# lixiaobai09/xgnn

Measured on AMD Instinct MI355X. Metric: sampled edges/s + feature-extract GB/s per epoch-step, higher is better.
Workload: dtype u32 ids / f32 rows (bit copy)

## Files before the change

### include/ggms.h

```cpp
#ifndef GGMS_H
#define GGMS_H

#include <stddef.h>
#include <stdint.h>

#ifdef __cplusplus
extern "C" {
#endif

typedef uint32_t ggms_id_t;
typedef void *ggms_stream_t;
typedef void *ggms_event_t;
#define GGMS_EMPTY_KEY 0xffffffffu

enum ggms_status {
  GGMS_OK = 0,
  GGMS_ERR_INVALID = -1,
  GGMS_ERR_HIP = -2,
  GGMS_ERR_NO_DEVICE = -3
};

enum ggms_dtype {
  GGMS_F32 = 0,
  GGMS_F64 = 1,
// ... 8 lines not shown
  GGMS_Q8ROW = 18
};

int ggms_abi_version(void);
const char *ggms_last_error(void);

#define GGMS_STATUS_SCAN_SPIN 1u
#define GGMS_STATUS_TABLE_FULL 2u
#define GGMS_STATUS_PREFETCH_FULL 4u
int ggms_device_status(uint32_t *status_host, int clear);
#define GGMS_PROBE_ATOMIC 0
#define GGMS_PROBE_LOAD 1
#define GGMS_PROBE_LOAD_ATOMIC 2
int ggms_fabric_probe(int kind, void *table, size_t table_words, size_t num_requests, uint32_t salt, void *sink,
                      ggms_stream_t stream);
void ggms_debug_poison_next_scan(void);
void ggms_debug_set_scan_patience(uint32_t polls);
void ggms_debug_delay_next_scan(uint32_t sleeps);
uint32_t ggms_debug_set_scan_epoch(uint32_t counter);
#define GGMS_DEBUG_KHOP0_DRAW_CAP 0
#define GGMS_DEBUG_OWNER_SCAN_CHUNKS 1
#define GGMS_DEBUG_OWNER_SCAN_TILES 2
#define GGMS_DEBUG_GRID_CAP 3
#define GGMS_DEBUG_NUM_KNOBS 4
void ggms_debug_set_knob(int knob, long long value);
size_t ggms_dtype_bytes(int dtype);
size_t ggms_row_bytes(int dtype, size_t dim);

#define GGMS_MAX_PARTS 8
typedef struct {
  const ggms_id_t *indptr;
  const ggms_id_t *indices;
  const ggms_id_t *const *part_indptr;
  const ggms_id_t *const *part_indices;
  uint32_t num_part;
  uint32_t num_cache_node;
  uint32_t num_node;
  uint32_t heads_id;
} ggms_graph_t;

#define GGMS_LIST_HEAD_BYTES 64
#define GGMS_LIST_HEAD_INLINE 15
#define GGMS_LIST_HEADS_MAX 255
size_t ggms_list_heads_bytes(size_t num_node);
int ggms_list_heads_build(const ggms_graph_t *graph, void *heads, size_t bytes, ggms_stream_t stream);
int ggms_list_heads_attach(ggms_graph_t *graph, const void *heads);
int ggms_list_heads_detach(ggms_graph_t *graph);
const void *ggms_list_heads_of(const ggms_graph_t *graph);
// ... 487 lines not shown
```

### xgnn_amd/_lib.py

```python
import ctypes as C
import os

_HERE = os.path.dirname(os.path.abspath(__file__))
LIB_PATH = os.path.join(_HERE, "lib", "libggms_hip.so")
_LIB = None


class GgmsError(RuntimeError):
    pass


class Graph(C.Structure):
    _fields_ = [("indptr", C.c_void_p), ("indices", C.c_void_p),
                ("part_indptr", C.c_void_p), ("part_indices", C.c_void_p),
                ("num_part", C.c_uint32), ("num_cache_node", C.c_uint32),
                ("num_node", C.c_uint32), ("heads_id", C.c_uint32)]


class SampleExtra(C.Structure):
    _fields_ = [("prob_table", C.c_void_p), ("alias_table", C.c_void_p), ("random_walk_length", C.c_size_t),
                ("random_walk_restart_prob", C.c_double), ("num_random_walk", C.c_size_t), ("data", C.c_void_p),
                ("rng_wait", C.c_void_p), ("rng_done", C.c_void_p), ("heavy_wait", C.c_void_p),
                ("seeds_distinct", C.c_uint32), ("labor_salt", C.c_uint32)]

# ... 57 lines not shown


class Topology(C.Structure):
    _fields_ = [("num_device", C.c_int32), ("_pad", C.c_int32), ("can_access", (C.c_int32 * 16) * 16),
                ("copy_GBps", (C.c_double * 16) * 16)]


class HashTable(C.Structure):
    _fields_ = [("o2n", C.c_void_p), ("n2o", C.c_void_p), ("num_items_dev", C.c_void_p),
                ("o2n_size", C.c_uint64), ("n2o_size", C.c_uint64),
                ("version", C.c_uint32), ("direct", C.c_uint32)]


_vp, _sz, _u64, _u32, _i = C.c_void_p, C.c_size_t, C.c_uint64, C.c_uint32, C.c_int
SYMBOLS = {
    "ggms_abi_version": (_i, []),
    "ggms_last_error": (C.c_char_p, []),
    "ggms_device_status": (_i, [C.POINTER(_u32), _i]),
    "ggms_debug_poison_next_scan": (None, []),
    "ggms_debug_set_scan_patience": (None, [C.c_uint32]),
    "ggms_debug_delay_next_scan": (None, [C.c_uint32]),
    "ggms_debug_set_scan_epoch": (C.c_uint32, [C.c_uint32]),
    "ggms_debug_set_knob": (None, [_i, C.c_longlong]),
    "ggms_fabric_probe": (_i, [_i, _vp, _sz, _sz, _u32, _vp, _vp]),
    "ggms_dtype_bytes": (_sz, [_i]),
    "ggms_row_bytes": (_sz, [_i, _sz]),
    "ggms_list_heads_bytes": (_sz, [_sz]),
    "ggms_list_heads_build": (_i, [C.POINTER(Graph), _vp, _sz, _vp]),
    "ggms_list_heads_attach": (_i, [C.POINTER(Graph), _vp]),
    "ggms_list_heads_detach": (_i, [C.POINTER(Graph)]),
    "ggms_list_heads_of": (_vp, [C.POINTER(Graph)]),
    "ggms_random_states_init": (_i, [_vp, _sz, _u64, _vp]),
    "ggms_random_states_count": (_sz, [_i, C.POINTER(_sz), _sz, _sz, _sz]),
    "ggms_sample_workspace_bytes": (_sz, [_i, _sz, _sz]),
    "ggms_sample_khop3": (_i, [C.POINTER(Graph), _vp, _sz, _sz, _vp, _vp, _vp, _vp, _sz, _vp, _sz, _vp]),
    "ggms_sample_khop0": (_i, [C.POINTER(Graph), _vp, _sz, _sz, _vp, _vp, _vp, _vp, _sz, _vp]),
    "ggms_sample_khop_labor": (_i, [C.POINTER(Graph), _vp, _sz, _sz, C.c_uint32, _vp, _vp, _vp, _vp, _sz, _vp]),
    "ggms_sample_khop_temporal": (_i, [C.POINTER(Graph), _vp, _vp, _vp, _sz, _sz, _i, C.c_uint32, _vp, _vp, _vp, _vp, _vp,
                                       _sz, _vp]),
    "ggms_sample_khop1": (_i, [C.POINTER(Graph), _vp, _sz, _sz, _vp, _vp, _vp, _vp, _sz, _vp, _sz, _vp]),
    "ggms_sample_khop2": (_i, [C.POINTER(Graph), _vp, _sz, _sz, _vp, _vp, _vp, _vp, _sz, _vp, _sz, _vp]),
    "ggms_sample_weighted_workspace_bytes": (_sz, [_sz, _sz]),
    "ggms_sample_weighted_khop": (_i, [C.POINTER(Graph), _vp, _vp, _vp, _sz, _sz, _vp, _vp, _vp, _vp, _sz, _vp, _sz,
                                       _vp]),
    "ggms_sample_weighted_khop_prefix": (_i, [C.POINTER(Graph), _vp, _vp, _sz, _sz, _vp, _vp, _vp, _vp, _sz, _vp, _sz,
                                              _vp]),
# ... 133 lines not shown
```

### xgnn_amd/csrc/common.hip

```cpp
#include <atomic>
#include <cstdarg>
#include <cstdio>
#include <mutex>
#include <random>

#include "row_formats.h"
#include "tile_scan.h"

namespace ggms {

static thread_local char g_err[512] = "";

void set_error(const char *fmt, ...) {
  va_list ap;
  va_start(ap, fmt);
  vsnprintf(g_err, sizeof(g_err), fmt, ap);
  va_end(ap);
}

uint32_t *device_status_word() {
  static std::mutex mu;
  static uint32_t *words[64] = {nullptr};
  int dev = 0;
  if (hipGetDevice(&dev) != hipSuccess || dev < 0 || dev >= 64) return nullptr;
  std::lock_guard<std::mutex> lock(mu);
  if (!words[dev]) {
    uint32_t *p = nullptr;
    if (hipMalloc((void **)&p, 64) != hipSuccess) return nullptr;
    if (hipMemset(p, 0, 64) != hipSuccess) {
      (void)hipFree(p);
      return nullptr;
    }
    words[dev] = p;
  }
  return words[dev];
}

size_t device_lds_bytes() {
  int dev = 0, v = 0;
  if (hipGetDevice(&dev) != hipSuccess) return 0;
  if (hipDeviceGetAttribute(&v, hipDeviceAttributeMaxSharedMemoryPerBlock, dev) != hipSuccess || v <= 0) return 0;
  return (size_t)v;
}

int raise_dynamic_lds(const void *func, size_t bytes, const char *who) {
  const size_t have = device_lds_bytes();
  if (have != 0 && bytes > have) {
    set_error("%s needs %zu bytes of LDS per workgroup, this device offers %zu: the library is built for gfx950 (160 KB)",
              who, bytes, have);
    return GGMS_ERR_INVALID;
  }
  GGMS_HIP(hipFuncSetAttribute(func, hipFuncAttributeMaxDynamicSharedMemorySize, (int)bytes));
  return GGMS_OK;
}

bool host_readable_table(const void *table, const char *what) {
  static thread_local const void *last_ok[2] = {nullptr, nullptr};
  if (table == last_ok[0] || table == last_ok[1]) return true;
  struct Remember {
    const void *t;
    bool ok = true;
    ~Remember() { if (ok) { last_ok[1] = last_ok[0]; last_ok[0] = t; } }
  } remember{table};
  hipPointerAttribute_t a;
  if (hipPointerGetAttributes(&a, table) != hipSuccess) {
    (void)hipGetLastError();
    return true;
  }
  if (a.type == hipMemoryTypeDevice) {
    set_error("%s is a DEVICE pointer: since ABI 3 the shard pointer tables are HOST arrays (include/ggms.h)", what);
    remember.ok = false;
    return false;
  }
  return true;
}

std::atomic<long long> &debug_knob_word(int knob) {
  static std::atomic<long long> v[GGMS_DEBUG_NUM_KNOBS] = {{-1}, {-1}, {-1}, {-1}};
  return v[knob];
}
long long debug_knob(int knob) { return debug_knob_word(knob).load(std::memory_order_relaxed); }

unsigned long long next_dedup_tag() {
  static std::atomic<unsigned long long> g{[] {
    std::random_device rd;
    return (((unsigned long long)rd() << 32) | rd()) | 1ull;
  }()};
  return g.fetch_add(1) + 1;
}

__global__ __launch_bounds__(kBlock) void k_init_states(uint32_t *states, uint64_t num, uint64_t seed) {
  for (uint64_t t = (uint64_t)blockIdx.x * kBlock + threadIdx.x; t < num; t += (uint64_t)gridDim.x * kBlock) {
    Xorwow st;
    st.init(seed + t);
    st.store(states + 6 * t);
  }
}

}

using namespace ggms;

extern "C" {

int ggms_abi_version(void) { return 3; }

void ggms_debug_set_knob(int knob, long long value) {
  if (knob >= 0 && knob < GGMS_DEBUG_NUM_KNOBS) debug_knob_word(knob).store(value < 0 ? -1 : value);
}

int ggms_device_status(uint32_t *status_host, int clear) {
  GGMS_CHECK_ARG(status_host);
  uint32_t *w = device_status_word();
  if (!w) {
    set_error("ggms_device_status: no device status word (no device?)");
    return GGMS_ERR_NO_DEVICE;
  }
  GGMS_HIP(hipDeviceSynchronize());
  GGMS_HIP(hipMemcpy(status_host, w, sizeof(uint32_t), hipMemcpyDeviceToHost));
  if (clear && *status_host) {
    GGMS_HIP(hipMemset(w, 0, sizeof(uint32_t)));
    GGMS_HIP(hipDeviceSynchronize());
  }
  return GGMS_OK;
}

const char *ggms_last_error(void) { return g_err; }

size_t ggms_dtype_bytes(int dtype) {
  switch (dtype) {
    case GGMS_F32: return 4;
    case GGMS_F64: return 8;
    case GGMS_F16: return 2;
    case GGMS_U8: return 1;
    case GGMS_I32: return 4;
    case GGMS_I8: return 1;
    case GGMS_I64: return 8;
    case GGMS_BF16: return 2;
    case GGMS_F8E4M3: return 1;
    case GGMS_F8E5M2: return 1;
    default: return 0;
  }
}

// ... 50 lines not shown
```

### xgnn_amd/csrc/ggms_device.h

```cpp
#pragma once
#include <cstdlib>

#include <hip/hip_runtime.h>
#include <stdint.h>

#include "../../include/ggms.h"

namespace ggms {

constexpr uint32_t kEmptyKey = GGMS_EMPTY_KEY;
constexpr int kWave = 64;
constexpr int kBlock = 256;
constexpr int kMaxGridBlocks = 2048;

void set_error(const char *fmt, ...);
#define GGMS_CHECK_ARG(cond)                                              \
  do {                                                                    \
    if (!(cond)) {                                                        \
      ::ggms::set_error("%s:%d: invalid argument: %s", __FILE__, __LINE__, #cond); \
      return GGMS_ERR_INVALID;                                            \
    }                                                                     \
  } while (0)
#define GGMS_HIP(call)                                                    \
  do {                                                                    \
// ... 194 lines not shown
  unsigned long long *w;
  uint32_t version;
  uint32_t *cand;
  unsigned long long *lost;
  unsigned long long tag;
  uint32_t base;
  uint32_t batch;
  IdxMap map;
  __device__ __forceinline__ unsigned long long issue(uint32_t key, uint32_t e) const {
    return atomicMin(w + key, make_w1(version, 1u, base + e));
  }
  __device__ __forceinline__ void enter(uint32_t key, uint32_t e) const { finish(issue(key, e), e); }
  __device__ __forceinline__ void finish(unsigned long long old, uint32_t e) const {
    const unsigned long long mine = make_w1(version, 1u, base + e);
    if (old > mine) {
      cand[e] = 1u;
      if ((old >> 32) == (mine >> 32)) lost[(uint32_t)old - base] = tag;
    } else {
      const uint32_t idx = (uint32_t)old;
      cand[e] = (batch && idx < base) ? 2u + map.local_of(idx) : 0u;
    }
  }
};
unsigned long long next_dedup_tag();
size_t device_lds_bytes();
int raise_dynamic_lds(const void *func, size_t bytes, const char *who);

__device__ __forceinline__ uint32_t lane_id() { return threadIdx.x & 63u; }

__device__ __forceinline__ uint64_t shfl_u64(uint64_t v, int src) {
  const uint32_t lo = __shfl((uint32_t)v, src, 64);
  const uint32_t hi = __shfl((uint32_t)(v >> 32), src, 64);
  return ((uint64_t)hi << 32) | lo;
}

__device__ __forceinline__ uint32_t wave_inclusive_scan(uint32_t x) {
#pragma unroll
  for (int off = 1; off < 64; off <<= 1) {
    const uint32_t y = __shfl_up(x, off, 64);
    if ((int)lane_id() >= off) x += y;
  }
  return x;
}

__device__ __forceinline__ uint32_t wave_reduce_sum(uint32_t x) {
#pragma unroll
// ... 23 lines not shown
```

### xgnn_amd/csrc/ggms_internal.h

```cpp
#pragma once
#include "tile_scan.h"

namespace ggms {

struct SrcMode {
  const uint32_t *seed_local;
  int local;
  __device__ __forceinline__ uint32_t value(uint32_t rid, uint64_t index) const {
    if (!local) return rid;
    return seed_local ? seed_local[index] : (uint32_t)index;
  }
};

struct BatchPrologue {
  uint32_t *zero_words;
  uint32_t num_zero;
  uint32_t *zero_words2;
  uint32_t num_zero2;
  uint32_t *num_items;
  uint64_t *record_n;
  uint32_t *zero_words3 = nullptr;
  uint32_t num_zero3 = 0;
  uint32_t items_are_seeds = 0;
  __device__ __forceinline__ void run(uint64_t n, uint32_t tid, uint32_t nthreads) const {
// ... 21 lines not shown
};
bool khop0_can_enter_seeds(size_t num_seeds);
size_t khop0_plan_desc_words(size_t num_seeds);

constexpr uint64_t kWeightedMaxThreads = 512 * 1024;
constexpr uint32_t kDedupSlots = 50;

struct SampleLayer {
  const ggms_graph_t *graph;
  const uint32_t *input;
  size_t n_max;
  size_t fanout;
  uint32_t *out_src, *out_dst;
  uint64_t *num_out;
  uint32_t *states, *workspace;
  hipStream_t s;
  Count n = {};
  GraphView g = {};
  SrcMode src = {};
  ScanArea *scan = nullptr;
  const DedupInsert *insert = nullptr;
  const FirstLayer *first = nullptr;
  const SeedEnter *enter = nullptr;
  const float *prob = nullptr;
  const uint32_t *alias = nullptr;
  uint32_t *out_data = nullptr;
  size_t walk_length = 0, num_walk = 0;
  double restart_prob = 0;
  uint32_t salt = 0;
  const uint32_t *edge_time = nullptr;
  const uint32_t *input_cut = nullptr;
  uint64_t *cut_table = nullptr;
  uint32_t stamp = 0;
  int pick = 0;
  uint32_t *out_pos = nullptr;
  const uint8_t *edge_type = nullptr;
  uint32_t num_type = 0;
  const uint32_t *type_fanout = nullptr;
  uint8_t *out_type = nullptr;
};

size_t sample_ws_words(size_t num_input);
size_t khop0_ws_words(size_t num_input, size_t fanout);
int sample_khop3_impl(const SampleLayer &l);
int sample_khop0_impl(const SampleLayer &l);
int sample_khop2_impl(const SampleLayer &l);
// ... 49 lines not shown
```

### xgnn_amd/csrc/sample_batch.hip

```cpp
#include <algorithm>
#include <functional>
#include <vector>

#include "ggms_internal.h"
#include "labor_hash.h"
#include "tile_scan.h"

namespace ggms {

__global__ void k_record(uint64_t *slot, Count c) {
  if (threadIdx.x == 0 && blockIdx.x == 0) *slot = c.get();
}

struct BatchCaps {
  size_t max_input[16];
  size_t max_edges[16];
  size_t max_in_all, max_e_all;
};

static BatchCaps caps_of(size_t num_seeds, const size_t *fanouts, uint32_t L) {
  BatchCaps c{};
  size_t n = num_seeds;
  for (int i = (int)L - 1; i >= 0; --i) {
    c.max_input[i] = n;
// ... 131 lines not shown
                               size_t *max_edges, size_t *max_unique) {
  GGMS_CHECK_ARG(fanouts && num_layer >= 1 && num_layer <= 16);
  const BatchCaps c = caps_of(num_seeds, fanouts, num_layer);
  for (uint32_t i = 0; i < num_layer; ++i) {
    if (max_input) max_input[i] = c.max_input[i];
    if (max_edges) max_edges[i] = c.max_edges[i];
  }
  if (max_unique) *max_unique = c.max_input[0] + c.max_edges[0];
  return GGMS_OK;
}

static size_t sampler_ws_words(int sample_type, const BatchCaps &c, const size_t *fanouts, uint32_t L,
                               const ggms_sample_extra_t *extra, size_t num_type) {
  size_t w = sample_ws_words(c.max_in_all);
  if (sample_type == GGMS_RANDOM_WALK && !extra) return w;
  for (uint32_t i = 0; i < L; ++i)
    w = std::max(w, layer_ws_words(sample_type, c.max_input[i], fanouts[i], extra ? extra->random_walk_length : 0,
                                   extra ? extra->num_random_walk : 0, num_type));
  return w;
}

struct BatchLayout {
  size_t seed_local, samp_ws, tmp_dst[16], cand, lost, scan, chunk, total;
  size_t pf_keys, pf_local, pf_pre, pf_scan, pf_total;
  size_t dedup_items;
  size_t scan_tiles;
};
static inline size_t up4(size_t w) { return (w + 3) & ~(size_t)3; }

static BatchLayout layout_of(int sample_type, size_t num_seeds, const size_t *fanouts, uint32_t L, const BatchCaps &c,
                             const ggms_sample_extra_t *extra, size_t pf_edges = 0, size_t num_type = 0) {
  BatchLayout l{};
  size_t w = 0;
  l.seed_local = w;  w += up4(num_seeds + 16);
  l.samp_ws = w;     w += up4(sampler_ws_words(sample_type, c, fanouts, L, extra, num_type));
  for (uint32_t i = 0; i < L; ++i) {
    l.tmp_dst[i] = w;
    w += up4(c.max_edges[i] + 16);
  }
  l.dedup_items = std::max({c.max_e_all, num_seeds, pf_edges});
  l.cand = w;        w += up4(l.dedup_items + 16);
  l.lost = w;        w += up4(2 * (l.dedup_items + 16));
  l.scan_tiles = std::max<size_t>({c.max_in_all / 128 + 2, owner_scan_tiles(l.dedup_items) + 2, kSinglePassTiles + 2});
  if (sample_type == GGMS_RANDOM_WALK) l.scan_tiles = std::max(l.scan_tiles, walk_scan_tiles(c.max_in_all));
  if (sample_type == GGMS_KHOP0) l.scan_tiles = std::max<size_t>(l.scan_tiles, 2 * (kSinglePassTiles + 2));
  l.scan = w;
  w += up4(std::max(tile_scan_words(std::max(c.max_e_all, c.max_in_all)), 8 + 2 * l.scan_tiles + 4) + 16);
  l.chunk = w;
  w += up4(chunk_desc_words() + (size_t)kTicketSets * kTicketWords);
  if (pf_edges) {
    l.pf_keys = w;   w += up4(pf_edges + 16);
    l.pf_local = w;  w += up4(pf_edges + 16);
    l.pf_pre = w;    w += up4(c.max_input[0] + 16);
    l.pf_scan = w;   w += up4(prefetch_scan_words(c.max_input[0]) + 16);
    l.pf_total = w;  w += 4;
  }
  l.total = w;
  return l;
}

size_t ggms_sample_batch_workspace_bytes(int sample_type, size_t num_seeds, const size_t *fanouts, uint32_t num_layer,
                                         const ggms_sample_extra_t *extra) {
  if (!fanouts || num_layer < 1 || num_layer > 16) return 0;
  const BatchCaps c = caps_of(num_seeds, fanouts, num_layer);
  return layout_of(sample_type, num_seeds, fanouts, num_layer, c, extra).total * sizeof(uint32_t) + 16;
}

struct Prefetch {
  size_t max_edges;
  hipEvent_t start, final;
};

// ... 94 lines not shown
      const size_t used = khop0_plan_desc_words(num_seeds);
      pro.num_zero = 8;
      pro.zero_words3 = pro.zero_words + 8 + used;
      pro.num_zero3 = (uint32_t)(2 * lay.scan_tiles > used ? 2 * lay.scan_tiles - used : 0);
      seed_enter = SeedEnter{(unsigned long long *)ht->o2n, ht->version, ht->n2o, pro};
    } else if (fuse_seeds) {
      const size_t tiles0 = (num_seeds + 127) / 128;
      pro.num_zero = 8;
      pro.zero_words3 = pro.zero_words + 8 + 2 * tiles0;
      pro.num_zero3 = (uint32_t)(lay.scan_tiles > tiles0 ? 2 * (lay.scan_tiles - tiles0) : 0);
      first_layer.pro = pro;
      first_layer.n2o = ht->n2o;
    } else {
      rc = seed_enter_impl(ht, seeds, num_seeds, pro, s);
    }
  } else {
    rc = ht_fill_impl(ht, seeds, num_seeds, count_of(num_seeds), di, false, scan, nullptr, nullptr, s, seed_local, &pro,
                      kRestNow, pro.record_n);
  }
  if (rc != GGMS_OK) return rc;
  if (tb) rc = temporal_seed_cut_impl(seeds, tb->seed_time, num_seeds, L.cut_table, L.stamp, s);
  if (rc != GGMS_OK) return rc;
  uint32_t next_base = (uint32_t)num_seeds;

  MapRestJobs jobs{};
  uint32_t num_jobs = 0;
  size_t job_items = 0;
  for (int i = (int)num_layer - 1; i >= 0; --i) {
    const bool first = (i == (int)num_layer - 1);
    const bool last_pf = pf && i == 0;
    uint32_t *tmp_dst = w + lay.tmp_dst[i];
    const size_t n_max = c.max_input[i], e_max = c.max_edges[i];
    uint64_t *num_dst0 = counts_dev + GGMS_COUNT_DST(0);
    const Count n = first ? count_of(num_seeds) : (last_pf ? count_of(n_max, num_dst0) : count_of32(n_max, ht->num_items_dev));
    uint64_t *num_edge = counts_dev + GGMS_COUNT_EDGES(i);
    uint64_t *num_src = counts_dev + GGMS_COUNT_SRC(i);
    uint64_t *next_dst = i > 0 ? counts_dev + GGMS_COUNT_DST(i - 1)
                               : counts_dev + GGMS_COUNT_INPUT(num_layer);
    if (first && ordered_rng && extra && extra->rng_wait) GGMS_HIP(hipStreamWaitEvent(s, (hipEvent_t)extra->rng_wait, 0));
    di.w = (unsigned long long *)ht->o2n;
    di.version = ht->version;
    if (last_pf) {
      if (pf->start) GGMS_HIP(hipEventRecord(pf->start, s));
      uint32_t *keys = w + lay.pf_keys, *local = w + lay.pf_local;
      uint64_t *total = reinterpret_cast<uint64_t *>(w + lay.pf_total);
      rc = prefetch_list_impl(L.g, ht->n2o, n_max, num_dst0, w + lay.pf_pre, w + lay.pf_scan, scan.status, total,
                              pf->max_edges, counts_dev + GGMS_COUNT_EXPANSION(num_layer), keys, s);
      if (rc != GGMS_OK) return rc;
      if (pf->max_edges == 0) {
        hipLaunchKernelGGL(k_record, dim3(1), dim3(64), 0, s, num_src, count_of32(0, ht->num_items_dev));
        hipLaunchKernelGGL(k_record, dim3(1), dim3(64), 0, s, next_dst, count_of32(0, ht->num_items_dev));
        GGMS_LAUNCH_CHECK();
      } else {
        di.base = next_base;
        rc = ht_fill_impl(ht, keys, pf->max_edges, count_of(pf->max_edges, total), di, false, scan, num_src, next_dst, s,
                          local, nullptr, kRestDefer, nullptr);
        if (rc != GGMS_OK) return rc;
        di.map.base[di.map.n] = next_base;
        di.map.arr[di.map.n] = local;
        ++di.map.n;
        next_base += (uint32_t)pf->max_edges;
      }
      if (pf->final) GGMS_HIP(hipEventRecord(pf->final, s));
    }
    if (i == 0 && extra && extra->heavy_wait) GGMS_HIP(hipStreamWaitEvent(s, (hipEvent_t)extra->heavy_wait, 0));
    di.base = next_base;
    const bool inserted = !last_pf && ht->direct != 0 && e_max != 0 && layer_enters_output(sample_type);
    if (inserted) di.tag = next_dedup_tag();
    if (n_max == 0) {
      GGMS_HIP(hipMemsetAsync(num_edge, 0, sizeof(uint64_t), s));
    } else {
      L.input = first ? seeds : ht->n2o;
      L.n_max = n_max;
      L.n = n;
      L.fanout = fanouts[i];
      L.salt = labor_layer_salt(extra ? extra->labor_salt : 0u, (uint32_t)i);
      L.out_src = col[i];
      L.out_dst = tmp_dst;
      L.num_out = num_edge;
      L.src = SrcMode{first ? seed_local : nullptr, 1};
      L.insert = inserted ? &di : nullptr;
      L.first = first && fuse_seeds ? &first_layer : nullptr;
      L.enter = first && khop0_enters ? &seed_enter : nullptr;
      if (sample_type == GGMS_RANDOM_WALK) L.out_data = extra->data[i];
      if (tb) L.out_pos = tb->eid[i];
      if (yb) {
        L.type_fanout = yb->t->type_fanout + (size_t)i * L.num_type;
        L.out_pos = yb->eid[i];
        L.out_type = yb->etype[i];
      }
      rc = sample_layer(sample_type, L);
    }
    if (rc != GGMS_OK) return rc;
    if (i == 0 && ordered_rng && extra && extra->rng_done) GGMS_HIP(hipEventRecord((hipEvent_t)extra->rng_done, s));
    const Count ne = count_of(e_max, num_edge);
    if (e_max == 0) {
      hipLaunchKernelGGL(k_record, dim3(1), dim3(64), 0, s, num_src, count_of32(0, ht->num_items_dev));
      hipLaunchKernelGGL(k_record, dim3(1), dim3(64), 0, s, next_dst, count_of32(0, ht->num_items_dev));
      GGMS_LAUNCH_CHECK();
      continue;
    }
    if (last_pf) {
      GGMS_HIP(hipMemsetAsync(row[i], 0xff, e_max * sizeof(uint32_t), s));
      jobs.row[num_jobs] = row[i];
      jobs.key[num_jobs] = tmp_dst;
      jobs.num[num_jobs] = num_edge;
      ++num_jobs;
      job_items = std::max(job_items, e_max);
      continue;
    }
    rc = ht_fill_impl(ht, tmp_dst, e_max, ne, di, inserted, scan, num_src, next_dst, s, row[i], nullptr,
                      ht->direct ? kRestDefer : kRestNow, nullptr);
    if (rc != GGMS_OK) return rc;
    if (ht->direct) {
      di.map.base[di.map.n] = next_base;
      di.map.arr[di.map.n] = row[i];
      ++di.map.n;
      next_base += (uint32_t)e_max;
      jobs.row[num_jobs] = row[i];
      jobs.key[num_jobs] = tmp_dst;
      jobs.num[num_jobs] = num_edge;
      ++num_jobs;
      job_items = std::max(job_items, e_max);
    }
  }
  if (tb) {
    rc = temporal_node_cut_impl(ht->n2o, c.max_input[0] + c.max_edges[0],
                                count_of32(c.max_input[0] + c.max_edges[0], ht->num_items_dev), L.cut_table, L.stamp,
                                tb->node_cut, s);
    if (rc != GGMS_OK) return rc;
  }
  return launch_map_rest_all(ht, jobs, num_jobs, job_items, di.map, counts_dev + GGMS_COUNT_STATUS(num_layer), s);
}

int ggms_sample_batch(int sample_type, const ggms_graph_t *graph, const ggms_id_t *seeds, size_t num_seeds,
                      const size_t *fanouts, uint32_t num_layer, ggms_hashtable_t *ht, void *states,
                      size_t num_states, ggms_id_t *const *row, ggms_id_t *const *col, uint64_t *counts_dev,
                      const ggms_sample_extra_t *extra, void *workspace, size_t workspace_bytes,
                      ggms_stream_t stream) {
  GGMS_CHECK_ARG(graph && fanouts && ht && row && col && counts_dev);
  GGMS_CHECK_ARG(num_layer >= 1 && num_layer <= 16);
  if (sample_type == GGMS_KHOP_TEMPORAL) {
    set_error("ggms_sample_batch: sample type %d (khop_temporal) takes edge times, seed times and a cut table: call "
              "ggms_sample_batch_temporal", sample_type);
    return GGMS_ERR_INVALID;
  }
// ... 152 lines not shown
```

### xgnn_amd/csrc/sample_khop.hip

```cpp
#include <algorithm>
#include <atomic>

#include "ggms_internal.h"

namespace ggms {

struct SeedCount {
  GraphView g;
  const uint32_t *input;
  uint32_t fanout;
  __device__ __forceinline__ uint32_t operator()(uint64_t i) const {
    uint32_t len;
    g.neighbours(input[i], len);
    return len < fanout ? len : fanout;
  }
};
struct StoreOffset {
  uint32_t *offset;
  __device__ __forceinline__ void operator()(uint64_t i, uint32_t, uint32_t excl) const { offset[i] = excl; }
};

template <int S>
__device__ __forceinline__ uint32_t row_shr(uint32_t v) {
  return (uint32_t)__builtin_amdgcn_update_dpp(0, (int)v, 0x110 + S, 0xf, 0xf, true);
// ... 2 lines not shown
template <bool HEADS>
struct Khop3TileHelp {
  static constexpr bool kCan = true;
  const GraphView &g;
  const uint32_t *input;
  uint64_t n;
  uint32_t fanout;
  __device__ __forceinline__ uint32_t operator()(uint64_t t) const {
    uint32_t acc = 0;
#pragma unroll
    for (uint32_t k = 0; k < 2; ++k) {
      const uint64_t i = 128 * t + 64 * k + (threadIdx.x & 63u);
      if (i < n) {
        uint32_t len;
        if constexpr (HEADS) len = g.heads[(uint64_t)input[i] * kHeadWords];
        else (void)g.neighbours(input[i], len);
        acc += len < fanout ? len : fanout;
      }
    }
    return wave_reduce_sum(acc);
  }
};

template <int GPW, bool INSERT, bool FIRST, bool HEADS>
__global__ __launch_bounds__(128 * (4 / GPW), 6) void k_khop3_fused(GraphView g, const uint32_t *__restrict__ input,
                                                                 Count n_arg, uint32_t fanout, uint32_t fanout_magic,
                                                                 uint32_t *__restrict__ out_src,
                                                                 uint32_t *__restrict__ out_dst, SrcMode sm,
                                                                 uint32_t *__restrict__ states, uint32_t set_mask,
                                                                 uint32_t multi, FusedScan fs, DedupInsert di,
                                                                 FirstLayer fl) {
  constexpr uint32_t HASH_EMPTY = 0xffffffffu, NT = 128 * (4 / GPW), FLAG_A = 1, FLAG_P = 2;
  extern __shared__ uint32_t s_pos[];
  __shared__ uint32_t set_tab[8][128];
  __shared__ const uint32_t *s_ptr[128];
  __shared__ uint32_t s_len[128], s_rid[128], s_off[129];
  __shared__ uint64_t s_tile;
  __shared__ uint32_t s_prefix;
  const uint32_t lane = threadIdx.x & 63u;
  const bool active = GPW == 4 || lane < 16u * GPW;
  const uint64_t n = n_arg.get();
  if constexpr (FIRST) {
    if (blockIdx.x == 0) fl.pro.run(n, threadIdx.x, NT);
  }
  const uint32_t y = (threadIdx.x >> 6) * GPW + (lane >> 4), lig = lane & 15u;
  const uint32_t grp_shift = lane & ~15u;
  uint32_t *const tab = set_tab[active ? y : 0];
  const uint64_t num_tiles = (n + 127) / 128;
  const uint32_t my_s = y + 8u * lig;
  uint32_t *const s_nbr = fanout >= kHeadInline ? s_pos : s_pos + 128u * fanout;
  const uint32_t nbr_stride = fanout >= kHeadInline ? fanout : kHeadInline;

  if (active)
    for (uint32_t s = lig; s <= set_mask; s += 16) tab[s] = HASH_EMPTY;
  bool dirty = false;

  const bool one_tile_each = gridDim.x >= num_tiles;
  for (uint32_t turn = 0;; ++turn) {
    if (one_tile_each) {
      if (turn != 0) break;
    } else {
      if (threadIdx.x == 0) s_tile = take_ticket(fs.tick);
      __syncthreads();
    }
    const uint64_t b = one_tile_each ? (uint64_t)blockIdx.x : s_tile;
    if (b >= num_tiles) break;
    uint32_t my_len = 0, my_magic = 0;
    unsigned long long seed_old = 0;
    if (active) {
      const uint64_t my_index = 128 * b + my_s;
      const uint32_t *ptr = nullptr;
      uint32_t rid = 0;
      if (my_index < n) {
        rid = input[my_index];
        if constexpr (FIRST) {
          fl.n2o[my_index] = rid;
          seed_old = atomicMin(di.w + rid, make_w1(di.version, 1u, (uint32_t)my_index));
        }
        if constexpr (HEADS) {
          const uint4 *rec = reinterpret_cast<const uint4 *>(g.heads + (uint64_t)rid * kHeadWords);
          const uint4 q0 = rec[0], q1 = rec[1], q2 = rec[2], q3 = rec[3];
          my_len = q0.x;
          if (my_len > kHeadInline) {
            ptr = g.indices + q0.y;
          } else if (my_len != 0) {
            uint32_t *d = s_nbr + my_s * nbr_stride;
            d[0] = q0.y; d[1] = q0.z; d[2] = q0.w;
            d[3] = q1.x; d[4] = q1.y; d[5] = q1.z; d[6] = q1.w;
            d[7] = q2.x; d[8] = q2.y; d[9] = q2.z; d[10] = q2.w;
            d[11] = q3.x; d[12] = q3.y; d[13] = q3.z; d[14] = q3.w;
          }
        } else {
          ptr = g.neighbours(rid, my_len);
        }
        if (my_len > fanout) my_magic = (uint32_t)(4294967296.0 / (double)my_len);
      }
      s_ptr[my_s] = ptr;
      s_len[my_s] = my_len;
      s_rid[my_s] = rid;
    }
    __syncthreads();
    if (threadIdx.x < kWave) {
      const uint32_t a = min(s_len[2 * lane], fanout), c = min(s_len[2 * lane + 1], fanout);
      const uint32_t incl = wave_inclusive_scan(a + c);
      s_off[2 * lane] = incl - (a + c);
      s_off[2 * lane + 1] = incl - c;
      if (lane == 63) {
        s_off[128] = incl;
        __hip_atomic_store(&fs.desc[b], scan_desc(fs.epoch, b == 0 ? FLAG_P : FLAG_A, incl), __ATOMIC_RELAXED,
                           __HIP_MEMORY_SCOPE_AGENT);
      }
    }
    if (active) {
      const uint64_t stream = 8 * b + y;
      const uint32_t my_off = my_s * fanout;
      uint32_t todo = (uint32_t)(__ballot(my_len > fanout) >> grp_shift) & 0xffffu;
      if (todo != 0) {
        Xorwow st;
        st.load(states + 6 * stream);
        bool fetch = true;
        uint32_t len = 0, o = 0, magic = 0, count = 0;
        while (todo != 0) {
// ... 88 lines not shown
        if (lig == 0) st.store(states + 6 * stream);
      }
    }
    if constexpr (FIRST) {
      const uint64_t my_index = 128 * b + my_s;
      if (active && my_index < n) {
        const unsigned long long mine = make_w1(di.version, 1u, (uint32_t)my_index);
        const uint32_t idx = (uint32_t)seed_old;
        if (seed_old > mine && (seed_old >> 32) == (mine >> 32) && idx >= di.base) di.lost[idx - di.base] = di.tag;
      }
    }
    if (threadIdx.x < kWave) {
      uint32_t prefix = 0;
      if (b != 0) {
        prefix = scan_lookback(fs.desc, b, fs.epoch, fs.err, fs.patience, Khop3TileHelp<HEADS>{g, input, n, fanout});
        if (lane == 0)
          __hip_atomic_store(&fs.desc[b], scan_desc(fs.epoch, FLAG_P, prefix + s_off[128]), __ATOMIC_RELAXED,
                             __HIP_MEMORY_SCOPE_AGENT);
      }
      if (lane == 0) {
        s_prefix = prefix;
        if (b + 1 == num_tiles) *fs.num_out = (uint64_t)prefix + s_off[128];
      }
    }
    __syncthreads();
    const uint32_t prefix = s_prefix;
    const uint32_t slots = 128u * fanout;
    const auto slot_of = [&](uint32_t t, uint32_t &sd, uint32_t &e, uint32_t &pos, bool &inl) -> bool {
      sd = fanout == 1 ? t : __umulhi(t, fanout_magic);
      if (sd * fanout > t) --sd;
      const uint32_t j = t - sd * fanout;
      const uint32_t len = s_len[sd];
      if (j >= (len < fanout ? len : fanout)) return false;
      e = prefix + s_off[sd] + j;
      pos = len <= fanout ? j : s_pos[t];
      inl = HEADS && len <= kHeadInline;
      return true;
    };
    const auto nbr_of = [&](uint32_t sd, uint32_t pos, bool inl) -> uint32_t {
      if constexpr (HEADS) {
        if (inl) return s_nbr[sd * nbr_stride + pos];
      }
      return s_ptr[sd][pos];
    };
    if (multi) {
      for (uint32_t t0 = threadIdx.x; t0 < slots; t0 += 4 * NT) {
        uint32_t sd[4], e[4], pos[4], nbr[4];
        bool ok[4], inl[4];
#pragma unroll
        for (uint32_t u = 0; u < 4; ++u) {
          const uint32_t t = t0 + u * NT;
          ok[u] = t < slots && slot_of(t, sd[u], e[u], pos[u], inl[u]);
          nbr[u] = ok[u] ? nbr_of(sd[u], pos[u], inl[u]) : 0u;
        }
        unsigned long long old[4];
#pragma unroll
        for (uint32_t u = 0; u < 4; ++u) {
          if (ok[u]) {
            out_src[e[u]] = sm.value(s_rid[sd[u]], 128 * b + sd[u]);
            out_dst[e[u]] = nbr[u];
            if (INSERT) old[u] = di.issue(nbr[u], e[u]);
          }
        }
        if (INSERT) {
#pragma unroll
          for (uint32_t u = 0; u < 4; ++u)
            if (ok[u]) di.finish(old[u], e[u]);
        }
      }
    } else {
      for (uint32_t t = threadIdx.x; t < slots; t += NT) {
        uint32_t sd, e, pos;
        bool inl;
        if (!slot_of(t, sd, e, pos, inl)) continue;
        const uint32_t nbr = nbr_of(sd, pos, inl);
        out_src[e] = sm.value(s_rid[sd], 128 * b + sd);
        out_dst[e] = nbr;
        if (INSERT) di.enter(nbr, e);
      }
    }
    __syncthreads();
  }
  if (threadIdx.x == 0 && num_tiles == 0 && blockIdx.x == 0) *fs.num_out = 0;
}

struct Khop0Count {
  GraphView g;
  const uint32_t *input;
  uint32_t fanout;
  __device__ __forceinline__ U2 operator()(uint64_t i) const {
    uint32_t len;
    g.neighbours(input[i], len);
    return len > fanout ? U2{fanout, len - fanout} : U2{len, 0u};
  }
};
struct Khop0Store {
  uint32_t *offset, *draw_base;
  unsigned long long *w;
  uint32_t version;
  const uint32_t *seeds;
  uint32_t *n2o;
  template <int CH>
  __device__ __forceinline__ void one(uint64_t i, uint32_t, uint32_t excl) const {
    (CH ? draw_base : offset)[i] = excl;
  }
  __device__ __forceinline__ void operator()(uint64_t i, uint32_t, uint32_t, uint32_t pa, uint32_t pb) const {
// ... 280 lines not shown
        tail[r] = len[r] - j - 1;
        picked[r] = indices[off[r] + sel[r]];
        moved[r] = indices[off[r] + tail[r]];
      }
#pragma unroll
      for (uint32_t r = 0; r < 4; ++r) {
        if (!draws[r]) continue;
        out_src[o[r] + j] = sv[r];
        out_dst[o[r] + j] = picked[r];
        indices[off[r] + sel[r]] = moved[r];
        indices[off[r] + tail[r]] = picked[r];
      }
    }
    st[3].store(states + 6 * sid);
  }
}

static int khop3_groups_per_wave(size_t blocks) { return blocks * 8 <= 2048 ? 1 : 2; }

size_t sample_ws_words(size_t num_input) {
  return num_input + tile_scan_words(num_input) + 16 + 2 * (num_input / 128 + 2) + kTicketWords + 16;
}

template <int GPW, bool INSERT, bool FIRST, bool HEADS>
static int launch_khop3_fused_h(int grid, size_t lds, const SampleLayer &l, uint32_t set_mask, uint32_t multi,
                                 FusedScan fs, DedupInsert di, FirstLayer fl) {
  const uint32_t fanout = (uint32_t)l.fanout;
  const uint32_t fanout_magic = (uint32_t)((0x100000000ull + fanout - 1) / fanout);
  if (lds > (48u << 10)) {
    static const int raised = raise_dynamic_lds(reinterpret_cast<const void *>(&k_khop3_fused<GPW, INSERT, FIRST, HEADS>),
                                                128 * 127 * 4, "k_khop3_fused (fanout >= 96)");
    if (raised != GGMS_OK) return raised;
  }
  hipLaunchKernelGGL((k_khop3_fused<GPW, INSERT, FIRST, HEADS>), dim3(grid), dim3(128 * (4 / GPW)), lds, l.s, l.g, l.input,
                     l.n, fanout, fanout_magic, l.out_src, l.out_dst, l.src, l.states, set_mask, multi, fs, di, fl);
  return GGMS_OK;
}

template <int GPW, bool INSERT, bool FIRST>
static int launch_khop3_fused(int grid, size_t lds, const SampleLayer &l, uint32_t set_mask, uint32_t multi,
                               FusedScan fs, DedupInsert di, FirstLayer fl) {
  if (l.g.heads) {
    if (l.fanout < kHeadInline) lds += 128 * kHeadInline * sizeof(uint32_t);
    return launch_khop3_fused_h<GPW, INSERT, FIRST, true>(grid, lds, l, set_mask, multi, fs, di, fl);
  }
  return launch_khop3_fused_h<GPW, INSERT, FIRST, false>(grid, lds, l, set_mask, multi, fs, di, fl);
}

bool khop3_can_fuse_seeds(size_t num_seeds) { return (num_seeds + 127) / 128 <= grid_cap(); }

int sample_khop3_impl(const SampleLayer &l) {
  ScanArea *shared_scan = l.scan;
  const DedupInsert *insert = l.insert;
  const FirstLayer *first = l.first;
  const size_t tiles = (l.n_max + 127) / 128;
  if (first && (!insert || !shared_scan || !shared_scan->cleared || !khop3_can_fuse_seeds(l.n_max))) {
    set_error("sample_khop3: the fused first layer needs the batch's dedup insert, its scan area and one tile per workgroup");
    return GGMS_ERR_INVALID;
  }
  uint32_t *ctl = scan_align(shared_scan ? shared_scan->words : l.workspace);
  uint32_t *tick = shared_scan ? take_ticket_set(shared_scan) : ctl + 8 + 2 * (tiles + 1) + 2;
  if (!tick) {
    set_error("sample_khop3: the shared scan area has no ticket set left");
    return GGMS_ERR_INVALID;
  }
  if (!shared_scan)
    GGMS_HIP(hipMemsetAsync(ctl, 0, (8 + 2 * (tiles + 1) + 2 + kTicketWords) * sizeof(uint32_t), l.s));
  else if (!shared_scan->cleared)
    GGMS_HIP(hipMemsetAsync(ctl, 0, (8 + 2 * (tiles + 1)) * sizeof(uint32_t), l.s));
  const FusedScan fs{tick, reinterpret_cast<unsigned long long *>(ctl + 8), next_scan_epoch(), l.num_out,
                     shared_scan ? shared_scan->status_word() : device_status_word(), scan_patience()};
  const uint32_t set_mask = l.fanout < 32 ? 63u : 127u;
  const int gpw = khop3_groups_per_wave(tiles);
  const int grid = grid_for(tiles, 1);
  const uint32_t multi = tiles <= grid_cap() ? 1u : 0u;
  const size_t lds = 128 * l.fanout * sizeof(uint32_t);
  const DedupInsert none{};
  const FirstLayer nofl{};
  int rc_l = GGMS_OK;
  if (first) {
    if (gpw == 1) rc_l = launch_khop3_fused<1, true, true>(grid, lds, l, set_mask, multi, fs, *insert, *first);
    else rc_l = launch_khop3_fused<2, true, true>(grid, lds, l, set_mask, multi, fs, *insert, *first);
  } else if (insert) {
    if (gpw == 1) rc_l = launch_khop3_fused<1, true, false>(grid, lds, l, set_mask, multi, fs, *insert, nofl);
    else rc_l = launch_khop3_fused<2, true, false>(grid, lds, l, set_mask, multi, fs, *insert, nofl);
  } else {
    if (gpw == 1) rc_l = launch_khop3_fused<1, false, false>(grid, lds, l, set_mask, multi, fs, none, nofl);
    else rc_l = launch_khop3_fused<2, false, false>(grid, lds, l, set_mask, multi, fs, none, nofl);
  }
  if (rc_l != GGMS_OK) return rc_l;
  GGMS_LAUNCH_CHECK();
  return GGMS_OK;
}

size_t khop0_draw_cap(size_t num_input, size_t fanout) {
  const unsigned long long want = 8ull * num_input * fanout;
  return (size_t)(want < 0x7fffffffull ? want : 0x7fffffffull);
}
bool khop0_can_enter_seeds(size_t num_seeds) { return scan2_single_launch(num_seeds); }
size_t khop0_plan_desc_words(size_t num_seeds) { return scan2_desc_words(num_seeds); }
size_t khop0_ws_words(size_t num_input, size_t fanout) {
  return 3 * num_input + tile_scan_words(num_input) + 48 + khop0_draw_cap(num_input, fanout);
}

int sample_khop0_impl(const SampleLayer &l) {
// ... 114 lines not shown
```

Before: 5.351 billion.

## Reuse earlier-layer dedup results for nodes whose full neighbour list was already taken

In k-hop (khop3) sampling with the direct dedup table, each layer now records per-input edge offsets. When a later layer's input node has degree no larger than an earlier layer's fanout, all its neighbours were already inserted, so the kernel reads the existing local ids from the earlier row output instead of running hash insert/finish. This cuts atomic dedup traffic on repeated nodes, at the cost of extra workspace, per-node lookups across earlier layers, extra template variants, and lower occupancy bounds for KD==3.

```diff
diff --git a/include/ggms.h b/include/ggms.h
--- a/include/ggms.h
+++ b/include/ggms.h
@@ -54,8 +54,11 @@
 #define GGMS_DEBUG_OWNER_SCAN_CHUNKS 1
 #define GGMS_DEBUG_OWNER_SCAN_TILES 2
 #define GGMS_DEBUG_GRID_CAP 3
-#define GGMS_DEBUG_NUM_KNOBS 4
+#define GGMS_DEBUG_KNOWN_DUPS_OFF 4
+#define GGMS_DEBUG_KNOWN_DUPS_COUNT 5
+#define GGMS_DEBUG_NUM_KNOBS 6
 void ggms_debug_set_knob(int knob, long long value);
+int ggms_debug_known_dups(uint64_t *count_host, int clear);
 size_t ggms_dtype_bytes(int dtype);
 size_t ggms_row_bytes(int dtype, size_t dim);
 
diff --git a/xgnn_amd/_lib.py b/xgnn_amd/_lib.py
--- a/xgnn_amd/_lib.py
+++ b/xgnn_amd/_lib.py
@@ -103,6 +103,7 @@
     "ggms_debug_delay_next_scan": (None, [C.c_uint32]),
     "ggms_debug_set_scan_epoch": (C.c_uint32, [C.c_uint32]),
     "ggms_debug_set_knob": (None, [_i, C.c_longlong]),
+    "ggms_debug_known_dups": (_i, [C.POINTER(_u64), _i]),
     "ggms_fabric_probe": (_i, [_i, _vp, _sz, _sz, _u32, _vp, _vp]),
     "ggms_dtype_bytes": (_sz, [_i]),
     "ggms_row_bytes": (_sz, [_i, _sz]),
diff --git a/xgnn_amd/csrc/common.hip b/xgnn_amd/csrc/common.hip
--- a/xgnn_amd/csrc/common.hip
+++ b/xgnn_amd/csrc/common.hip
@@ -36,6 +36,24 @@
   return words[dev];
 }
 
+unsigned long long *known_dups_counter() {
+  static std::mutex mu;
+  static unsigned long long *words[64] = {nullptr};
+  int dev = 0;
+  if (hipGetDevice(&dev) != hipSuccess || dev < 0 || dev >= 64) return nullptr;
+  std::lock_guard<std::mutex> lock(mu);
+  if (!words[dev]) {
+    unsigned long long *p = nullptr;
+    if (hipMalloc((void **)&p, 64) != hipSuccess) return nullptr;
+    if (hipMemset(p, 0, 64) != hipSuccess) {
+      (void)hipFree(p);
+      return nullptr;
+    }
+    words[dev] = p;
+  }
+  return words[dev];
+}
+
 size_t device_lds_bytes() {
   int dev = 0, v = 0;
   if (hipGetDevice(&dev) != hipSuccess) return 0;
@@ -76,7 +94,7 @@
 }
 
 std::atomic<long long> &debug_knob_word(int knob) {
-  static std::atomic<long long> v[GGMS_DEBUG_NUM_KNOBS] = {{-1}, {-1}, {-1}, {-1}};
+  static std::atomic<long long> v[GGMS_DEBUG_NUM_KNOBS] = {{-1}, {-1}, {-1}, {-1}, {-1}, {-1}};
   return v[knob];
 }
 long long debug_knob(int knob) { return debug_knob_word(knob).load(std::memory_order_relaxed); }
@@ -120,6 +138,22 @@
   GGMS_HIP(hipMemcpy(status_host, w, sizeof(uint32_t), hipMemcpyDeviceToHost));
   if (clear && *status_host) {
     GGMS_HIP(hipMemset(w, 0, sizeof(uint32_t)));
+    GGMS_HIP(hipDeviceSynchronize());
+  }
+  return GGMS_OK;
+}
+
+int ggms_debug_known_dups(uint64_t *count_host, int clear) {
+  GGMS_CHECK_ARG(count_host);
+  unsigned long long *w = known_dups_counter();
+  if (!w) {
+    set_error("ggms_debug_known_dups: no device counter (no device?)");
+    return GGMS_ERR_NO_DEVICE;
+  }
+  GGMS_HIP(hipDeviceSynchronize());
+  GGMS_HIP(hipMemcpy(count_host, w, sizeof(uint64_t), hipMemcpyDeviceToHost));
+  if (clear) {
+    GGMS_HIP(hipMemset(w, 0, sizeof(uint64_t)));
     GGMS_HIP(hipDeviceSynchronize());
   }
   return GGMS_OK;
diff --git a/xgnn_amd/csrc/ggms_device.h b/xgnn_amd/csrc/ggms_device.h
--- a/xgnn_amd/csrc/ggms_device.h
+++ b/xgnn_amd/csrc/ggms_device.h
@@ -240,6 +240,17 @@
     }
   }
 };
+struct KnownLayers {
+  uint32_t n;
+  uint32_t fanout[16];
+  const uint64_t *inputs[16];
+  const uint32_t *edge_off[16];
+  const uint32_t *row[16];
+  uint32_t *edge_off_out;
+  unsigned long long *counter;
+};
+unsigned long long *known_dups_counter();
+
 unsigned long long next_dedup_tag();
 size_t device_lds_bytes();
 int raise_dynamic_lds(const void *func, size_t bytes, const char *who);
diff --git a/xgnn_amd/csrc/ggms_internal.h b/xgnn_amd/csrc/ggms_internal.h
--- a/xgnn_amd/csrc/ggms_internal.h
+++ b/xgnn_amd/csrc/ggms_internal.h
@@ -67,6 +67,7 @@
   const DedupInsert *insert = nullptr;
   const FirstLayer *first = nullptr;
   const SeedEnter *enter = nullptr;
+  const KnownLayers *known = nullptr;
   const float *prob = nullptr;
   const uint32_t *alias = nullptr;
   uint32_t *out_data = nullptr;
diff --git a/xgnn_amd/csrc/sample_batch.hip b/xgnn_amd/csrc/sample_batch.hip
--- a/xgnn_amd/csrc/sample_batch.hip
+++ b/xgnn_amd/csrc/sample_batch.hip
@@ -177,6 +177,7 @@
 
 struct BatchLayout {
   size_t seed_local, samp_ws, tmp_dst[16], cand, lost, scan, chunk, total;
+  size_t edge_off[16];
   size_t pf_keys, pf_local, pf_pre, pf_scan, pf_total;
   size_t dedup_items;
   size_t scan_tiles;
@@ -203,6 +204,11 @@
   w += up4(std::max(tile_scan_words(std::max(c.max_e_all, c.max_in_all)), 8 + 2 * l.scan_tiles + 4) + 16);
   l.chunk = w;
   w += up4(chunk_desc_words() + (size_t)kTicketSets * kTicketWords);
+  if (sample_type == GGMS_KHOP3)
+    for (uint32_t i = 1; i < L; ++i) {
+      l.edge_off[i] = w;
+      w += up4(c.max_input[i] + 16);
+    }
   if (pf_edges) {
     l.pf_keys = w;   w += up4(pf_edges + 16);
     l.pf_local = w;  w += up4(pf_edges + 16);
@@ -343,6 +349,10 @@
   if (tb) rc = temporal_seed_cut_impl(seeds, tb->seed_time, num_seeds, L.cut_table, L.stamp, s);
   if (rc != GGMS_OK) return rc;
   uint32_t next_base = (uint32_t)num_seeds;
+  const bool known_dups = sample_type == GGMS_KHOP3 && ht->direct != 0 && !pf && num_layer >= 2 &&
+                          debug_knob(GGMS_DEBUG_KNOWN_DUPS_OFF) <= 0;
+  KnownLayers known{};
+  if (known_dups && debug_knob(GGMS_DEBUG_KNOWN_DUPS_COUNT) > 0) known.counter = known_dups_counter();
 
   MapRestJobs jobs{};
   uint32_t num_jobs = 0;
@@ -388,6 +398,8 @@
     di.base = next_base;
     const bool inserted = !last_pf && ht->direct != 0 && e_max != 0 && layer_enters_output(sample_type);
     if (inserted) di.tag = next_dedup_tag();
+    L.known = nullptr;
+    known.edge_off_out = nullptr;
     if (n_max == 0) {
       GGMS_HIP(hipMemsetAsync(num_edge, 0, sizeof(uint64_t), s));
     } else {
@@ -403,6 +415,10 @@
       L.insert = inserted ? &di : nullptr;
       L.first = first && fuse_seeds ? &first_layer : nullptr;
       L.enter = first && khop0_enters ? &seed_enter : nullptr;
+      if (known_dups && inserted && (i > 0 || known.n != 0)) {
+        known.edge_off_out = i > 0 && (!first || distinct) ? w + lay.edge_off[i] : nullptr;
+        if (known.edge_off_out || known.n != 0) L.known = &known;
+      }
       if (sample_type == GGMS_RANDOM_WALK) L.out_data = extra->data[i];
       if (tb) L.out_pos = tb->eid[i];
       if (yb) {
@@ -443,6 +459,13 @@
       jobs.num[num_jobs] = num_edge;
       ++num_jobs;
       job_items = std::max(job_items, e_max);
+      if (L.known && known.edge_off_out) {
+        known.fanout[known.n] = (uint32_t)fanouts[i];
+        known.inputs[known.n] = counts_dev + GGMS_COUNT_DST(i);
+        known.edge_off[known.n] = known.edge_off_out;
+        known.row[known.n] = row[i];
+        ++known.n;
+      }
     }
   }
   if (tb) {
diff --git a/xgnn_amd/csrc/sample_khop.hip b/xgnn_amd/csrc/sample_khop.hip
--- a/xgnn_amd/csrc/sample_khop.hip
+++ b/xgnn_amd/csrc/sample_khop.hip
@@ -48,14 +48,15 @@
   }
 };
 
-template <int GPW, bool INSERT, bool FIRST, bool HEADS>
-__global__ __launch_bounds__(128 * (4 / GPW), 6) void k_khop3_fused(GraphView g, const uint32_t *__restrict__ input,
+template <int GPW, bool INSERT, bool FIRST, bool HEADS, int KD>
+__global__ __launch_bounds__(128 * (4 / GPW), KD == 3 ? 5 : 6) void k_khop3_fused(GraphView g, const uint32_t *__restrict__ input,
                                                                  Count n_arg, uint32_t fanout, uint32_t fanout_magic,
                                                                  uint32_t *__restrict__ out_src,
                                                                  uint32_t *__restrict__ out_dst, SrcMode sm,
                                                                  uint32_t *__restrict__ states, uint32_t set_mask,
                                                                  uint32_t multi, FusedScan fs, DedupInsert di,
-                                                                 FirstLayer fl) {
+                                                                 FirstLayer fl, KnownLayers kl) {
+  static_assert(KD == 0 || INSERT, "known duplicates belong to a batch with the direct table");
   constexpr uint32_t HASH_EMPTY = 0xffffffffu, NT = 128 * (4 / GPW), FLAG_A = 1, FLAG_P = 2;
   extern __shared__ uint32_t s_pos[];
   __shared__ uint32_t set_tab[8][128];
@@ -63,7 +64,12 @@
   __shared__ uint32_t s_len[128], s_rid[128], s_off[129];
   __shared__ uint64_t s_tile;
   __shared__ uint32_t s_prefix;
+  __shared__ const uint32_t *s_known[KD >= 2 ? 128 : 1];
+  __shared__ uint32_t s_count;
   const uint32_t lane = threadIdx.x & 63u;
+  if constexpr (KD >= 2) {
+    if (threadIdx.x == 0) s_count = 0;
+  }
   const bool active = GPW == 4 || lane < 16u * GPW;
   const uint64_t n = n_arg.get();
   if constexpr (FIRST) {
@@ -93,11 +99,21 @@
     if (b >= num_tiles) break;
     uint32_t my_len = 0, my_magic = 0;
     unsigned long long seed_old = 0;
+    uint32_t known_inst = 0;
     if (active) {
       const uint64_t my_index = 128 * b + my_s;
       const uint32_t *ptr = nullptr;
+      const uint32_t *known = nullptr;
       uint32_t rid = 0;
       if (my_index < n) {
+        uint32_t known_off = 0;
+        bool was_input = false;
+        if constexpr (KD >= 2) {
+          if (kl.n != 0 && my_index < *kl.inputs[kl.n - 1]) {
+            was_input = true;
+            known_off = kl.edge_off[kl.n - 1][my_index];
+          }
+        }
         rid = input[my_index];
         if constexpr (FIRST) {
           fl.n2o[my_index] = rid;
@@ -120,10 +136,34 @@
           ptr = g.neighbours(rid, my_len);
         }
         if (my_len > fanout) my_magic = (uint32_t)(4294967296.0 / (double)my_len);
-      }
+        if constexpr (KD >= 2) {
+          if (was_input && my_len != 0) {
+            if (my_len <= kl.fanout[kl.n - 1]) {
+              known = kl.row[kl.n - 1] + known_off;
+            } else {
+              const uint32_t *eo = nullptr, *rw = nullptr;
+#pragma unroll 1
+              for (uint32_t k = 0; k + 1 < kl.n; ++k) {
+                const bool ok = my_index < *kl.inputs[k] && my_len <= kl.fanout[k];
+                eo = ok ? kl.edge_off[k] : eo;
+                rw = ok ? kl.row[k] : rw;
+              }
+              if (rw != nullptr) known = rw + eo[my_index];
+            }
+            if (known != nullptr) known_inst = my_len < fanout ? my_len : fanout;
+          }
+        }
+      }
+      if constexpr (KD >= 2) s_known[my_s] = known;
       s_ptr[my_s] = ptr;
       s_len[my_s] = my_len;
       s_rid[my_s] = rid;
+    }
+    if constexpr (KD >= 2) {
+      if (kl.counter) {
+        const uint32_t t = wave_reduce_sum(known_inst);
+        if (lane == 0 && t != 0) atomicAdd(&s_count, t);
+      }
     }
     __syncthreads();
     if (threadIdx.x < kWave) {
@@ -258,6 +298,13 @@
         s_prefix = prefix;
         if (b + 1 == num_tiles) *fs.num_out = (uint64_t)prefix + s_off[128];
       }
+      if constexpr (KD != 0) {
+        if (kl.edge_off_out != nullptr) {
+          const uint64_t i = 128 * b + 2 * lane;
+          if (i < n) kl.edge_off_out[i] = prefix + s_off[2 * lane];
+          if (i + 1 < n) kl.edge_off_out[i + 1] = prefix + s_off[2 * lane + 1];
+        }
+      }
     }
     __syncthreads();
     const uint32_t prefix = s_prefix;
@@ -279,7 +326,7 @@
       }
       return s_ptr[sd][pos];
     };
-    if (multi) {
+    if (multi && KD != 2) {
       for (uint32_t t0 = threadIdx.x; t0 < slots; t0 += 4 * NT) {
         uint32_t sd[4], e[4], pos[4], nbr[4];
         bool ok[4], inl[4];
@@ -295,13 +342,27 @@
           if (ok[u]) {
             out_src[e[u]] = sm.value(s_rid[sd[u]], 128 * b + sd[u]);
             out_dst[e[u]] = nbr[u];
-            if (INSERT) old[u] = di.issue(nbr[u], e[u]);
+            if constexpr (KD == 3) {
+              const uint32_t *known = s_known[sd[u]];
+              old[u] = known != nullptr ? (unsigned long long)known[pos[u]] : di.issue(nbr[u], e[u]);
+            } else if (INSERT) {
+              old[u] = di.issue(nbr[u], e[u]);
+            }
           }
         }
         if (INSERT) {
 #pragma unroll
-          for (uint32_t u = 0; u < 4; ++u)
-            if (ok[u]) di.finish(old[u], e[u]);
+          for (uint32_t u = 0; u < 4; ++u) {
+            if (!ok[u]) continue;
+            if constexpr (KD == 3) {
+              if ((old[u] >> 32) == 0) {
+                const uint32_t id = (uint32_t)old[u];
+                di.cand[e[u]] = id != kEmptyKey ? 2u + id : 0u;
+                continue;
+              }
+            }
+            di.finish(old[u], e[u]);
+          }
         }
       }
     } else {
@@ -312,12 +373,26 @@
         const uint32_t nbr = nbr_of(sd, pos, inl);
         out_src[e] = sm.value(s_rid[sd], 128 * b + sd);
         out_dst[e] = nbr;
-        if (INSERT) di.enter(nbr, e);
+        if constexpr (KD >= 2) {
+          const uint32_t *known = s_known[sd];
+          if (known != nullptr) {
+            const uint32_t id = known[pos];
+            di.cand[e] = id != kEmptyKey ? 2u + id : 0u;
+          } else {
+            di.enter(nbr, e);
+          }
+        } else if (INSERT) {
+          di.enter(nbr, e);
+        }
       }
     }
     __syncthreads();
   }
   if (threadIdx.x == 0 && num_tiles == 0 && blockIdx.x == 0) *fs.num_out = 0;
+  if constexpr (KD >= 2) {
+    if (threadIdx.x == 0 && kl.counter != nullptr && s_count != 0)
+      atomicAdd(kl.counter, (unsigned long long)s_count);
+  }
 }
 
 struct Khop0Count {
@@ -644,29 +719,30 @@
   return num_input + tile_scan_words(num_input) + 16 + 2 * (num_input / 128 + 2) + kTicketWords + 16;
 }
 
-template <int GPW, bool INSERT, bool FIRST, bool HEADS>
+template <int GPW, bool INSERT, bool FIRST, bool HEADS, int KD>
 static int launch_khop3_fused_h(int grid, size_t lds, const SampleLayer &l, uint32_t set_mask, uint32_t multi,
-                                 FusedScan fs, DedupInsert di, FirstLayer fl) {
+                                 FusedScan fs, DedupInsert di, FirstLayer fl, const KnownLayers &kl) {
   const uint32_t fanout = (uint32_t)l.fanout;
   const uint32_t fanout_magic = (uint32_t)((0x100000000ull + fanout - 1) / fanout);
   if (lds > (48u << 10)) {
-    static const int raised = raise_dynamic_lds(reinterpret_cast<const void *>(&k_khop3_fused<GPW, INSERT, FIRST, HEADS>),
+    static const int raised = raise_dynamic_lds(reinterpret_cast<const void *>(&k_khop3_fused<GPW, INSERT, FIRST, HEADS, KD>),
                                                 128 * 127 * 4, "k_khop3_fused (fanout >= 96)");
     if (raised != GGMS_OK) return raised;
   }
-  hipLaunchKernelGGL((k_khop3_fused<GPW, INSERT, FIRST, HEADS>), dim3(grid), dim3(128 * (4 / GPW)), lds, l.s, l.g, l.input,
-                     l.n, fanout, fanout_magic, l.out_src, l.out_dst, l.src, l.states, set_mask, multi, fs, di, fl);
+  hipLaunchKernelGGL((k_khop3_fused<GPW, INSERT, FIRST, HEADS, KD>), dim3(grid), dim3(128 * (4 / GPW)), lds, l.s, l.g,
+                     l.input, l.n, fanout, fanout_magic, l.out_src, l.out_dst, l.src, l.states, set_mask, multi, fs, di, fl,
+                     kl);
   return GGMS_OK;
 }
 
-template <int GPW, bool INSERT, bool FIRST>
+template <int GPW, bool INSERT, bool FIRST, int KD = 0>
 static int launch_khop3_fused(int grid, size_t lds, const SampleLayer &l, uint32_t set_mask, uint32_t multi,
-                               FusedScan fs, DedupInsert di, FirstLayer fl) {
+                               FusedScan fs, DedupInsert di, FirstLayer fl, const KnownLayers &kl = KnownLayers{}) {
   if (l.g.heads) {
     if (l.fanout < kHeadInline) lds += 128 * kHeadInline * sizeof(uint32_t);
-    return launch_khop3_fused_h<GPW, INSERT, FIRST, true>(grid, lds, l, set_mask, multi, fs, di, fl);
-  }
-  return launch_khop3_fused_h<GPW, INSERT, FIRST, false>(grid, lds, l, set_mask, multi, fs, di, fl);
+    return launch_khop3_fused_h<GPW, INSERT, FIRST, true, KD>(grid, lds, l, set_mask, multi, fs, di, fl, kl);
+  }
+  return launch_khop3_fused_h<GPW, INSERT, FIRST, false, KD>(grid, lds, l, set_mask, multi, fs, di, fl, kl);
 }
 
 bool khop3_can_fuse_seeds(size_t num_seeds) { return (num_seeds + 127) / 128 <= grid_cap(); }
@@ -700,9 +776,22 @@
   const DedupInsert none{};
   const FirstLayer nofl{};
   int rc_l = GGMS_OK;
-  if (first) {
+  if (l.known && !insert) {
+    set_error("sample_khop3: the known-duplicates descriptor needs the batch's dedup insert");
+    return GGMS_ERR_INVALID;
+  }
+  if (first && l.known) {
+    if (gpw == 1) rc_l = launch_khop3_fused<1, true, true, 1>(grid, lds, l, set_mask, multi, fs, *insert, *first, *l.known);
+    else rc_l = launch_khop3_fused<2, true, true, 1>(grid, lds, l, set_mask, multi, fs, *insert, *first, *l.known);
+  } else if (first) {
     if (gpw == 1) rc_l = launch_khop3_fused<1, true, true>(grid, lds, l, set_mask, multi, fs, *insert, *first);
     else rc_l = launch_khop3_fused<2, true, true>(grid, lds, l, set_mask, multi, fs, *insert, *first);
+  } else if (l.known && multi) {
+    if (gpw == 1) rc_l = launch_khop3_fused<1, true, false, 3>(grid, lds, l, set_mask, multi, fs, *insert, nofl, *l.known);
+    else rc_l = launch_khop3_fused<2, true, false, 3>(grid, lds, l, set_mask, multi, fs, *insert, nofl, *l.known);
+  } else if (l.known) {
+    if (gpw == 1) rc_l = launch_khop3_fused<1, true, false, 2>(grid, lds, l, set_mask, multi, fs, *insert, nofl, *l.known);
+    else rc_l = launch_khop3_fused<2, true, false, 2>(grid, lds, l, set_mask, multi, fs, *insert, nofl, *l.known);
   } else if (insert) {
     if (gpw == 1) rc_l = launch_khop3_fused<1, true, false>(grid, lds, l, set_mask, multi, fs, *insert, nofl);
     else rc_l = launch_khop3_fused<2, true, false>(grid, lds, l, set_mask, multi, fs, *insert, nofl);
```

After: 5.306 billion. No clear change (-0.8%).
